# IlzeAmandaA/VAE-GP-ODE

Hardware: AMD Instinct MI355X
Metric: latent_trajectories_per_sec (higher is better)
Workload: dtype f32; 1 GPU; configs[1]: ode1 DF q=6 M=100 S=256 T=16 batch=256; step = full ELBO training step (encoder, GP draw, rk4 rollout, decoder, ELBO, backward, Adam), L=1; global_batch=256, mc_draws=1, solver=rk4 (3/8 rule), parallelism=dp1, hip_graph=True, graph_scope=whole, gp_side_stream=True, batchnorm=per-process statistics

## Files before the change

vae-gp-ode_amd/csrc/gp_cache.hip:

```cpp
#include <type_traits>
#include "gp_eval.hpp"
#include "gp_launch.hpp"
#include "wave_reduce.hpp"
#include "gp_ws.hpp"

namespace gp {

static constexpr float kJitter = 1e-5f;

__device__ __forceinline__ float softplus_lower(float x) {
  float sp = x > 20.f ? x : log1pf(expf(x));
  return sp + 1e-12f;
}

struct PrepArgs {
  int kernel, Di, Do, M, S;
  const float *raw_ell, *raw_var, *Z, *Um, *Us, *eps_u, *rff_w, *rff_eps, *rff_u;
  float *pack, *pack_ind, *uni;
  float *ell_ws, *var_ws, *u_ws;
  float *ell_out, *var_out, *omega_out, *phase_out, *u_out;
  int* info;
  int nb_rff, nb_u, nb_ind, nb_hyp, nb_om;
  size_t s_eps_u, s_rff_w, s_rff_eps, s_rff_u, s_pack;
};
// ... 228 lines not shown
  return bad;
}

__global__ __launch_bounds__(256) void k_chol_rl(float* __restrict__ Aall, float* __restrict__ Lall, int np,
                                                  size_t batch_stride, float* __restrict__ Dfac_all, size_t dfac_stride,
                                                  int k, int* __restrict__ info, int nblk, int jlim, int nreal) {
  __shared__ float sD[NB][NB + 1], sI[NB][NB + 1], sJ[NB][NB + 1];
  __shared__ float lD[NB][NB + 1], lI[NB][NB + 1], lJ[NB][NB + 1];
  float* A = Aall + (size_t)blockIdx.y * batch_stride;
  float* Lm = Lall + (size_t)blockIdx.y * batch_stride;
  float* Dfac = Dfac_all + (size_t)blockIdx.y * dfac_stride + (size_t)k * NB * NB;
  const int t = blockIdx.x;
  int i, j;
  if (jlim >= nblk) {
    int ii = (int)((sqrtf(8.f * (float)t + 1.f) - 1.f) * 0.5f);
    while ((ii + 1) * (ii + 2) / 2 <= t) ++ii;
    while (ii * (ii + 1) / 2 > t) --ii;
    i = k + ii; j = k + (t - ii * (ii + 1) / 2);
  } else {
    int rem = t;
    j = k;
    while (rem >= nblk - j) { rem -= nblk - j; ++j; }
    i = j + rem;
  }
  const bool hasI = i > k, hasJ = (j > k) && (j != i);
  const int tid = threadIdx.x, tx = tid & 31, ty = tid >> 5;
  const int c0 = k * NB;
#pragma unroll
  for (int q = 0; q < 4; ++q) {
    const int r = ty + 8 * q;
    sD[r][tx] = A[(size_t)(c0 + r) * np + c0 + tx];
    sI[r][tx] = hasI ? A[(size_t)(i * NB + r) * np + c0 + tx] : 0.f;
    sJ[r][tx] = hasJ ? A[(size_t)(j * NB + r) * np + c0 + tx] : 0.f;
  }
  __syncthreads();
  const int wv = tid >> 6, lane = tid & 63;
  if (wv == 0 || (wv == 1 && hasJ)) {
    const int r = lane & 31;
    const bool panel = lane >= 32;
    float row[NB];
#pragma unroll
    for (int c = 0; c < NB; ++c) row[c] = panel ? (wv == 0 ? sI[r][c] : sJ[r][c]) : sD[r][c];
    const bool bad = chol32_panel_wave(row);
    if (bad && wv == 0 && t == 0 && lane == 0) atomicOr(info, 1);
    float* dst = panel ? (wv == 0 ? &lI[r][0] : &lJ[r][0]) : &lD[r][0];
#pragma unroll
    for (int c = 0; c < NB; ++c) dst[c] = (panel || c <= r) ? row[c] : 0.f;
  }
  __syncthreads();
  if (j == k) {
#pragma unroll
    for (int q = 0; q < 4; ++q) {
      const int r = ty + 8 * q;
      if (i == k) {
        Dfac[r * NB + tx] = lD[r][tx];
        if (r == tx && c0 + r < nreal) {
          atomicMin(reinterpret_cast<unsigned*>(info) + 1, __float_as_uint(lD[r][tx]));
          atomicMax(reinterpret_cast<unsigned*>(info) + 2, __float_as_uint(lD[r][tx]));
        }
      } else Lm[(size_t)(i * NB + r) * np + c0 + tx] = lI[r][tx];
    }
  } else {
#pragma unroll
    for (int q = 0; q < 4; ++q) {
      const int r = ty + 8 * q;
      float acc = 0.f;
      if (hasJ) {
#pragma unroll 8
        for (int p = 0; p < NB; ++p) acc = fmaf(lI[r][p], lJ[tx][p], acc);
      } else {
#pragma unroll 8
        for (int p = 0; p < NB; ++p) acc = fmaf(lI[r][p], lI[tx][p], acc);
      }
      float* dst = A + (size_t)(i * NB + r) * np + j * NB + tx;
      *dst = *dst - acc;
    }
  }
}

__device__ __forceinline__ void tile_load(float (&dst)[NB][NB + 1], const float* __restrict__ A, int np, int r0, int c0, int tx, int ty) {
#pragma unroll
  for (int q = 0; q < 4; ++q) dst[ty + 8 * q][tx] = A[(size_t)(r0 + ty + 8 * q) * np + c0 + tx];
}
__device__ __forceinline__ void tile_sub_xyt(float (&dst)[NB][NB + 1], const float (&src)[NB][NB + 1], const float (&X)[NB][NB + 1],
                                             const float (&Y)[NB][NB + 1], int tx, int ty) {
#pragma unroll
  for (int q = 0; q < 4; ++q) {
    const int r = ty + 8 * q;
    float acc = 0.f;
#pragma unroll 8
    for (int p = 0; p < NB; ++p) acc = fmaf(X[r][p], Y[tx][p], acc);
    dst[r][tx] = src[r][tx] - acc;
  }
}
__device__ __forceinline__ bool tile_factor(const float (&Dt)[NB][NB + 1], const float (&Pt)[NB][NB + 1], float (&Lp)[NB][NB + 1],
                                            float (*Ld)[NB + 1], int lane) {
  const int r = lane & 31;
  const bool panel = lane >= 32;
  float row[NB];
#pragma unroll
  for (int c = 0; c < NB; ++c) row[c] = panel ? Pt[r][c] : Dt[r][c];
  const bool bad = chol32_panel_wave(row);
  if (panel) {
#pragma unroll
    for (int c = 0; c < NB; ++c) Lp[r][c] = row[c];
  } else if (Ld) {
#pragma unroll
    for (int c = 0; c < NB; ++c) Ld[r][c] = c <= r ? row[c] : 0.f;
  }
  return bad;
}

__global__ __launch_bounds__(256) void k_chol_rl2(float* __restrict__ Aall, float* __restrict__ Lall, int np, size_t batch_stride,
                                                   float* __restrict__ Dfac_all, size_t dfac_stride, int k, int* __restrict__ info,
                                                   int nblk, int nreal) {
  __shared__ float sD[NB][NB + 1], sPi[NB][NB + 1], sPj[NB][NB + 1], sP1[NB][NB + 1];
  __shared__ float sE[NB][NB + 1], sQi[NB][NB + 1], sQj[NB][NB + 1];
  __shared__ float lD[NB][NB + 1], lPi[NB][NB + 1], lPj[NB][NB + 1], lP1[NB][NB + 1];
  __shared__ float lE[NB][NB + 1], lQi[NB][NB + 1], lQj[NB][NB + 1];
  float* A = Aall + (size_t)blockIdx.y * batch_stride;
  float* Lm = Lall + (size_t)blockIdx.y * batch_stride;
  float* DfacB = Dfac_all + (size_t)blockIdx.y * dfac_stride;
  const int t = blockIdx.x;
  int ii = (int)((sqrtf(8.f * (float)t + 1.f) - 1.f) * 0.5f);
  while ((ii + 1) * (ii + 2) / 2 <= t) ++ii;
  while (ii * (ii + 1) / 2 > t) --ii;
  const int i = k + ii, j = k + (t - ii * (ii + 1) / 2);
  const int k1 = k + 1;
  const int tid = threadIdx.x, tx = tid & 31, ty = tid >> 5, wv = tid >> 6, lane = tid & 63;
  const int c0 = k * NB, c1 = k1 * NB;
  const bool colk = j == k;
  const bool colk1 = j == k1;
  const bool needI = i > k, needJ = j > k && j != i;
  const bool need1 = !colk && i != k1 && j != k1;
  tile_load(sD, A, np, c0, c0, tx, ty);
  if (needI) tile_load(sPi, A, np, i * NB, c0, tx, ty);
  if (needJ) tile_load(sPj, A, np, j * NB, c0, tx, ty);
  if (need1) tile_load(sP1, A, np, c1, c0, tx, ty);
  if (!colk) {
    tile_load(sE, A, np, c1, c1, tx, ty);
    if (i > k1) tile_load(sQi, A, np, i * NB, c1, tx, ty);
    if (j > k1 && j != i) tile_load(sQj, A, np, j * NB, c1, tx, ty);
  }
  __syncthreads();
  bool bad = false;
  if (wv == 0) bad = tile_factor(sD, needI ? sPi : sD, lPi, lD, lane);
  else if (wv == 1 && needJ) tile_factor(sD, sPj, lPj, nullptr, lane);
  else if (wv == 2 && need1) tile_factor(sD, sP1, lP1, nullptr, lane);
  if (bad && t == 0 && lane == 0 && wv == 0) atomicOr(info, 1);
  __syncthreads();
  if (colk) {
#pragma unroll
    for (int q = 0; q < 4; ++q) {
      const int r = ty + 8 * q;
      if (i == k) {
        DfacB[(size_t)k * NB * NB + r * NB + tx] = lD[r][tx];
        if (r == tx && c0 + r < nreal) {
          atomicMin(reinterpret_cast<unsigned*>(info) + 1, __float_as_uint(lD[r][tx]));
          atomicMax(reinterpret_cast<unsigned*>(info) + 2, __float_as_uint(lD[r][tx]));
        }
      } else Lm[(size_t)(i * NB + r) * np + c0 + tx] = lPi[r][tx];
    }
    return;
  }
  const float (&L1)[NB][NB + 1] = (i == k1) ? lPi : ((j == k1) ? lPj : lP1);
  tile_sub_xyt(sE, sE, L1, L1, tx, ty);
  if (i > k1) tile_sub_xyt(sQi, sQi, lPi, L1, tx, ty);
  if (j > k1 && j != i) tile_sub_xyt(sQj, sQj, lPj, L1, tx, ty);
  __syncthreads();
  bool bad1 = false;
  if (wv == 0) bad1 = tile_factor(sE, i > k1 ? sQi : sE, lQi, lE, lane);
  else if (wv == 1 && j > k1 && j != i) tile_factor(sE, sQj, lQj, nullptr, lane);
  if (bad1 && t == 2 && lane == 0 && wv == 0) atomicOr(info, 1);
  __syncthreads();
  if (colk1) {
#pragma unroll
    for (int q = 0; q < 4; ++q) {
      const int r = ty + 8 * q;
      if (i == k1) {
        DfacB[(size_t)k1 * NB * NB + r * NB + tx] = lE[r][tx];
        if (r == tx && c1 + r < nreal) {
          atomicMin(reinterpret_cast<unsigned*>(info) + 1, __float_as_uint(lE[r][tx]));
          atomicMax(reinterpret_cast<unsigned*>(info) + 2, __float_as_uint(lE[r][tx]));
        }
      } else Lm[(size_t)(i * NB + r) * np + c1 + tx] = lQi[r][tx];
    }
    return;
  }
  const float (&Lj0)[NB][NB + 1] = (j == i) ? lPi : lPj;
  const float (&Lj1)[NB][NB + 1] = (j == i) ? lQi : lQj;
#pragma unroll
  for (int q = 0; q < 4; ++q) {
    const int r = ty + 8 * q;
    float acc = 0.f;
#pragma unroll 8
    for (int p = 0; p < NB; ++p) acc = fmaf(lPi[r][p], Lj0[tx][p], acc);
#pragma unroll 8
    for (int p = 0; p < NB; ++p) acc = fmaf(lQi[r][p], Lj1[tx][p], acc);
    float* dst = A + (size_t)(i * NB + r) * np + j * NB + tx;
    *dst = *dst - acc;
  }
}

typedef float cf32x4 __attribute__((ext_vector_type(4)));
constexpr int ST = 128, SK = 16, SLD = ST + 16;

__global__ __launch_bounds__(256, 2) void k_syrk_mfma(float* __restrict__ Aall, const float* __restrict__ Lall, int np,
                                                       size_t batch_stride, int r0, int c0) {
  __shared__ __attribute__((aligned(16))) float sA[SK][SLD], sB[SK][SLD];
  float* A = Aall + (size_t)blockIdx.y * batch_stride;
  const float* Lm = Lall + (size_t)blockIdx.y * batch_stride;
  const int t = blockIdx.x;
  int tm = (int)((sqrtf(8.f * (float)t + 1.f) - 1.f) * 0.5f);
  while ((tm + 1) * (tm + 2) / 2 <= t) ++tm;
  while (tm * (tm + 1) / 2 > t) --tm;
  const int tn = t - tm * (tm + 1) / 2;
  const int tid = threadIdx.x, lane = tid & 63, wave = tid >> 6, lr = lane & 15, lk = lane >> 4;
  const int wm = (wave & 1) * 64, wn = (wave >> 1) * 64;
  cf32x4 acc[4][4];
#pragma unroll
  for (int i = 0; i < 4; ++i)
#pragma unroll
    for (int j = 0; j < 4; ++j) acc[i][j] = cf32x4{0.f, 0.f, 0.f, 0.f};
  const float* Pa = Lm + ((size_t)r0 + (size_t)tm * ST) * np + c0;
  const float* Pb = Lm + ((size_t)r0 + (size_t)tn * ST) * np + c0;
  float4 ra[2], rb[2];
  auto load = [&](int kt) {
#pragma unroll
    for (int q = 0; q < 2; ++q) {
      const int e = tid + 256 * q, m = e >> 2, k4 = (e & 3) * 4;
      ra[q] = *reinterpret_cast<const float4*>(&Pa[(size_t)m * np + kt * SK + k4]);
      rb[q] = *reinterpret_cast<const float4*>(&Pb[(size_t)m * np + kt * SK + k4]);
    }
  };
  load(0);
  for (int kt = 0; kt < ST / SK; ++kt) {
    __syncthreads();
#pragma unroll
    for (int q = 0; q < 2; ++q) {
      const int e = tid + 256 * q, m = e >> 2, k4 = (e & 3) * 4;
      sA[k4 + 0][m] = ra[q].x; sA[k4 + 1][m] = ra[q].y; sA[k4 + 2][m] = ra[q].z; sA[k4 + 3][m] = ra[q].w;
      sB[k4 + 0][m] = rb[q].x; sB[k4 + 1][m] = rb[q].y; sB[k4 + 2][m] = rb[q].z; sB[k4 + 3][m] = rb[q].w;
    }
    __syncthreads();
    if (kt + 1 < ST / SK) load(kt + 1);
#pragma unroll
    for (int ks = 0; ks < SK / 4; ++ks) {
      float af[4], bf[4];
#pragma unroll
      for (int i = 0; i < 4; ++i) { af[i] = sA[4 * ks + lk][wm + 16 * i + lr]; bf[i] = sB[4 * ks + lk][wn + 16 * i + lr]; }
#pragma unroll
      for (int i = 0; i < 4; ++i)
#pragma unroll
        for (int j = 0; j < 4; ++j) acc[i][j] = __builtin_amdgcn_mfma_f32_16x16x4f32(af[i], bf[j], acc[i][j], 0, 0, 0);
    }
  }
  float* C = A + ((size_t)r0 + (size_t)tm * ST) * np + r0 + (size_t)tn * ST;
#pragma unroll
  for (int i = 0; i < 4; ++i)
#pragma unroll
    for (int j = 0; j < 4; ++j)
#pragma unroll
      for (int r = 0; r < 4; ++r) {
        float* dst = C + (size_t)(wm + 16 * i + 4 * lk + r) * np + wn + 16 * j + lr;
        *dst = *dst - acc[i][j][r];
      }
}

template <int CP4>
__global__ __launch_bounds__(256) void k_solve_back(const float* __restrict__ Aall, int n, int np, size_t batch_stride,
                                                     const float* __restrict__ Dfac_all, size_t dfac_stride,
                                                     const float* __restrict__ u, int u_stride, int u_bstride,
                                                     float* __restrict__ nu, float* __restrict__ nu_out,
                                                     int kernel, int Di, int Do, int M, const float* __restrict__ var,
                                                     float* __restrict__ pack_ind, size_t u_dstride, size_t nu_dstride,
                                                     size_t pack_dstride) {
  extern __shared__ __attribute__((aligned(16))) float sv[];
  __shared__ float sx[NB];
  const int b = blockIdx.x, dr = blockIdx.y;
  const float* A = Aall + (size_t)b * batch_stride;
  const float* Dfac = Dfac_all + (size_t)b * dfac_stride;
  u += (size_t)dr * u_dstride;
  nu += (size_t)dr * nu_dstride;
// ... 487 lines not shown
  }
  if (c != P) {
    if (half == 0) y[col] = res;
    return;
  }
  float colv[PW];
  const int g0 = P * PW;
  if (half == 0) {
#pragma unroll
    for (int r = 0; r < PW; ++r) colv[r] = (r >= tid && g0 + r < n) ? factor_elem(Lm, Dfac, np, g0 + r, g0 + tid) : 0.f;
  }
  __syncthreads();
#pragma unroll
  for (int r = PW - 1; r >= 0; --r) {
    if (tid == r) {
      const float x = (g0 + r < n) ? res / colv[r] : 0.f;
      sx[r] = x;
      res = x;
    }
    __syncthreads();
    if (tid < r) res = fmaf(-colv[r], sx[r], res);
  }
  if (half == 0 && col < n) nub[col] = res;
}

__global__ void k_nu_publish(int n, const float* __restrict__ nu, float* __restrict__ nu_out, int kernel, int Di, int Do,
                             const float* __restrict__ var, float* __restrict__ pack_ind, size_t nu_dstride, size_t pack_dstride) {
  const int b = blockIdx.y, j = blockIdx.x * blockDim.x + threadIdx.x;
  if (j >= n) return;
  nu += (size_t)blockIdx.z * nu_dstride;
  if (nu_out) nu_out += (size_t)blockIdx.z * nu_dstride;
  pack_ind += (size_t)blockIdx.z * pack_dstride;
  const float v = nu[(size_t)b * n + j];
  if (nu_out) nu_out[(size_t)b * n + j] = v;
  if (!pack_ind) return;
  const int RQ2 = cdiv(Di + Do, 4);
  int m, d;
  float coef;
  if (kernel == 0) { m = j; d = b; coef = var[d] * v; } else { m = j / Do; d = j % Do; coef = v; }
  const int field = Di + d;
  pack_ind[(((size_t)(m >> 6) * RQ2 + (field >> 2)) * 64 + (m & 63)) * 4 + (field & 3)] = coef;
}

__global__ void k_fill_from_K(int kernel, int Do, int n, int np, const float* __restrict__ Ku, const float* __restrict__ u_prior,
                              float* __restrict__ A) {
  const int c = blockIdx.x * blockDim.x + threadIdx.x;
  const int r = blockIdx.y, b = blockIdx.z;
  if (c >= np) return;
  float v;
  if (r < n && c < n) v = Ku[((size_t)b * n + r) * n + c] + (r == c ? kJitter : 0.f);
  else if (r == n) v = c < n ? (kernel == 0 ? u_prior[(size_t)c * Do + b] : u_prior[c]) : (c == n ? 1e30f : 0.f);
  else v = (r == c) ? 1.f : 0.f;
  A[((size_t)b * np + r) * np + c] = v;
}

__global__ void k_copy_L(const float* __restrict__ Aall, const float* __restrict__ Dfac_all, size_t dinv_stride,
                         int n, int np, size_t batch_stride, float* __restrict__ Lu) {
  const int c = blockIdx.x * blockDim.x + threadIdx.x;
  const int r = blockIdx.y, b = blockIdx.z;
  if (c >= n) return;
  float v = 0.f;
  if (c <= r) {
    const int kb = r / NB;
    v = (c < kb * NB) ? Aall[(size_t)b * batch_stride + (size_t)r * np + c]
                      : Dfac_all[(size_t)b * dinv_stride + ((size_t)kb * NB + (r - kb * NB)) * NB + (c - kb * NB)];
  }
  Lu[((size_t)b * n + r) * n + c] = v;
}

static size_t pack_floats_for(int kernel, int Di, int Do, int M, int S) {
  const size_t SJ = cdiv(S, 64), MJ = cdiv(M, 64);
  if (kernel == 0) return 256 * (SJ * Do * cdiv(Di + 2, 4) + MJ * cdiv(Di + Do, 4)) + (size_t)cdiv(Do * Di, 4) * 4;
  return 256 * (SJ * Do * cdiv(2 * Do + 3, 4) + MJ * cdiv(2 * Do, 4)) + (size_t)cdiv(2 * Do * Do + Do, 4) * 4;
}

int cache_sizes(int kernel, int Di, int Do, int M, int S, size_t* pack_floats, size_t* ws_floats, int nd) {
  if (!dims_supported(kernel, Di, Do)) return set_error("gpode_cache_sizes: no specialisation for kernel=%d Di=%d Do=%d", kernel, Di, Do);
  if (M < 1 || S < 1 || nd < 1) return set_error("gpode_cache_sizes: M=%d S=%d draws=%d", M, S, nd);
  if (pack_floats) *pack_floats = pack_floats_for(kernel, Di, Do, M, S);
  if (ws_floats) *ws_floats = ws_layout(kernel, Di, Do, M, S, nd).total;
  return 0;
}

static void cholesky_blocked(float* A, float* Lmat, float* Dfac, int np, int nblk, int batch, int* info, hipStream_t st, int nreal) {
  struct { int np, nblk, batch; } w{np, nblk, batch};
  const size_t bstride = (size_t)np * np, dstride = (size_t)nblk * NB * NB;
  constexpr int PB = ST / NB;
  if (big_factor(w.np)) {
    for (int K = 0; K < w.nblk / PB; ++K) {
      const int jlim = (K + 1) * PB;
      for (int k = K * PB; k < jlim; ++k) {
        int tiles = 0;
        for (int j = k; j < jlim; ++j) tiles += w.nblk - j;
        hipLaunchKernelGGL(k_chol_rl, dim3(tiles, w.batch), 256, 0, st, A, Lmat, w.np, bstride, Dfac, dstride, k, info, w.nblk, jlim, nreal);
      }
      const int Tt = w.nblk / PB - (K + 1);
      if (Tt > 0)
        hipLaunchKernelGGL(k_syrk_mfma, dim3(Tt * (Tt + 1) / 2, w.batch), 256, 0, st, A, Lmat, w.np, bstride, jlim * NB, K * ST);
    }
  } else {
    int k = 0;
    for (; k + 1 < w.nblk; k += 2) {
      const int T = w.nblk - k;
      hipLaunchKernelGGL(k_chol_rl2, dim3(T * (T + 1) / 2, w.batch), 256, 0, st, A, Lmat, w.np, bstride, Dfac, dstride, k, info, w.nblk, nreal);
    }
    for (; k < w.nblk; ++k) {
      const int T = w.nblk - k;
      hipLaunchKernelGGL(k_chol_rl, dim3(T * (T + 1) / 2, w.batch), 256, 0, st, A, Lmat, w.np, bstride, Dfac, dstride, k, info, w.nblk, w.nblk, nreal);
    }
  }
}

int cache_build_fwd(int kernel, int Di, int Do, int M, int S, int nd,
                    const float* raw_ell, const float* raw_var, const float* Z, const float* Um, const float* Us_packed,
                    const float* eps_u, const float* rff_w, const float* rff_eps, const float* rff_u,
                    float* pack, float* ws, float* ell, float* var, float* omega, float* phase, float* u,
                    float* Lu, float* nu, float* u_prior, hipStream_t st) {
  if (!dims_supported(kernel, Di, Do)) return set_error("gpode_cache_build_fwd: no specialisation for kernel=%d Di=%d Do=%d", kernel, Di, Do);
  if (kernel == 1 && Di != Do) return set_error("gpode_cache_build_fwd: DF needs D_in == D_out (kernels.py:259-262)");
  if (nd < 1 || nd > 65535) return set_error("gpode_cache_build_fwd: %d draws", nd);
  const WsLayout w = ws_layout(kernel, Di, Do, M, S, nd);
  const size_t SJ = cdiv(S, 64), MJ = cdiv(M, 64);
  const size_t rff_f4 = (kernel == 0 ? SJ * Do * cdiv(Di + 2, 4) : SJ * Do * cdiv(2 * Do + 3, 4)) * 64;
  const size_t ind_f4 = (kernel == 0 ? MJ * cdiv(Di + Do, 4) : MJ * cdiv(2 * Do, 4)) * 64;
  const size_t pf = pack_floats_for(kernel, Di, Do, M, S);
  const size_t MD = (size_t)M * Do;
  float* pack_ind = pack + 4 * rff_f4;
  float* uni = pack + 4 * (rff_f4 + ind_f4);
  int* info = reinterpret_cast<int*>(ws + w.info);
  {
    PrepArgs a;
    a.kernel = kernel; a.Di = Di; a.Do = Do; a.M = M; a.S = S;
    a.raw_ell = raw_ell; a.raw_var = raw_var; a.Z = Z; a.Um = Um; a.Us = Us_packed;
    a.eps_u = eps_u; a.rff_w = rff_w; a.rff_eps = rff_eps; a.rff_u = rff_u;
    a.pack = pack; a.pack_ind = pack_ind; a.uni = uni;
    a.ell_ws = ws + w.ell; a.var_ws = ws + w.var; a.u_ws = ws + w.u;
    a.ell_out = ell; a.var_out = var; a.omega_out = omega; a.phase_out = phase; a.u_out = u;
    a.info = info;
    a.nb_rff = cdiv((int)(SJ * Do * 64), 256);
    a.nb_u = cdiv(M * Do, 4);
    a.nb_ind = cdiv((int)(MJ * 64), 256);
    a.nb_hyp = 1;
    a.nb_om = (omega || phase) ? cdiv(Di * S * Do, 256) : 0;
    a.s_eps_u = MD; a.s_rff_w = (size_t)(kernel == 0 ? S : 2 * S) * Do; a.s_rff_eps = (size_t)Di * S * Do; a.s_rff_u = (size_t)S * Do;
    a.s_pack = pf;
    hipLaunchKernelGGL(k_prep, dim3(a.nb_rff + a.nb_u + a.nb_ind + a.nb_hyp + a.nb_om, nd), 256, 0, st, a);
    if (check_launch("cache prep")) return 1;
  }

  float* up = u_prior ? u_prior : ws + w.u_prior;
  if (rhs_fwd(kernel, Di, Do, M, S, pack, Z, M, up, 1, st, Draws{nd, pf, 0, MD})) return 1;

  float* A = ws + w.A;
  float* Lmat = ws + w.Lmat;
  float* Dfac = ws + w.Dfac;
  const size_t bstride = (size_t)w.np * w.np, dstride = (size_t)w.nblk * NB * NB;
  if (draw_in_lds(w.np, M, Di, nd)) {
    const size_t lds = draw_lds_bytes(w.np, M, Di, nd);
    if (kernel == 0) {
      if (set_max_lds((const void*)k_draw_lds<0>, lds)) return 1;
      hipLaunchKernelGGL(k_draw_lds<0>, w.batch, 512, lds, st, Di, Do, M, w.n, w.np, w.nblk, Z, ws + w.ell, ws + w.var, up, ws + w.u, Lmat,
                         bstride, Dfac, dstride, ws + w.nu, nu, pack_ind, info, nd, MD, MD, pf);
    } else {
      if (set_max_lds((const void*)k_draw_lds<1>, lds)) return 1;
      hipLaunchKernelGGL(k_draw_lds<1>, w.batch, 512, lds, st, Di, Do, M, w.n, w.np, w.nblk, Z, ws + w.ell, ws + w.var, up, ws + w.u, Lmat,
                         bstride, Dfac, dstride, ws + w.nu, nu, pack_ind, info, nd, MD, MD, pf);
    }
    if (Lu) hipLaunchKernelGGL(k_copy_L, dim3(cdiv(w.n, 128), w.n, w.batch), 128, 0, st, Lmat, Dfac, dstride, w.n, w.np, bstride, Lu);
    return check_launch("cache build: lds");
  }
  if (kernel == 0)
    hipLaunchKernelGGL(k_Kzz_rbf, dim3(cdiv(w.np, 128), w.np, Do), 128, 0, st, Di, Do, M, w.np, Z, ws + w.ell, ws + w.var, up, A, nd);
  else
    hipLaunchKernelGGL(k_Kzz_df, dim3(cdiv(w.np, 128), w.np, 1), 128, 0, st, Do, M, w.np, Z, ws + w.ell, ws + w.var, up, A, nd);
  cholesky_blocked(A, Lmat, Dfac, w.np, w.nblk, w.batch, info, st, w.n);
  if (check_launch("cholesky")) return 1;

  const int u_stride = kernel == 0 ? Do : 1, u_bstride = kernel == 0 ? 1 : 0;
  const char* route = "cache build: panel";
  if (big_factor(w.np)) {
    const int npanel = cdiv(w.n, ST);
    for (int P = npanel - 1; P >= 0; --P)
      hipLaunchKernelGGL(k_solve_back_panel, dim3(P + 1, w.batch, nd), 256, 0, st, Lmat, w.n, w.np, bstride, Dfac, dstride, ws + w.u,
                         u_stride, u_bstride, A, ws + w.nu, P, P == npanel - 1 ? 1 : 0, MD, MD);
    hipLaunchKernelGGL(k_nu_publish, dim3(cdiv(w.n, 256), w.batch, nd), 256, 0, st, w.n, ws + w.nu, nu, kernel, Di, Do, ws + w.var, pack_ind,
                       MD, pf);
  } else {
    if (solve_back_deep_fits(w.np, w.nblk)) {
      const size_t ldsd = sizeof(float) * ((size_t)w.np + (size_t)w.nblk * NB * NB);
      if (set_max_lds((const void*)k_solve_back_deep, ldsd)) return 1;
      hipLaunchKernelGGL(k_solve_back_deep, dim3(w.batch, nd), SBD_THREADS, ldsd, st, Lmat, w.n, w.np, bstride, Dfac, dstride, ws + w.u,
                         u_stride, u_bstride, ws + w.nu, nu, kernel, Di, Do, M, ws + w.var, pack_ind, MD, MD, pf);
      if (Lu) hipLaunchKernelGGL(k_copy_L, dim3(cdiv(w.n, 128), w.n, w.batch), 128, 0, st, Lmat, Dfac, dstride, w.n, w.np, bstride, Lu);
      return check_launch("cache build: chain32+deep");
    }
    const size_t lds = sizeof(float) * w.np;
    const int cpt = cdiv(w.n, 1024);
#define GP_SOLVE(CPT)                                                                                              \
  do {                                                                                                             \
    if (set_max_lds((const void*)k_solve_back<CPT>, lds)) return 1;                                                \
    hipLaunchKernelGGL(k_solve_back<CPT>, dim3(w.batch, nd), 256, lds, st, Lmat, w.n, w.np, bstride, Dfac, dstride, ws + w.u,   \
                       u_stride, u_bstride, ws + w.nu, nu, kernel, Di, Do, M, ws + w.var, pack_ind, MD, MD, pf);   \
  } while (0)
    if (cpt == 1) GP_SOLVE(1);
    else if (cpt == 2) GP_SOLVE(2);
    else GP_SOLVE(0);
#undef GP_SOLVE
    route = cpt == 1 ? "cache build: chain32+back<1>" : cpt == 2 ? "cache build: chain32+back<2>" : "cache build: chain32+back<0>";
  }
  if (Lu) hipLaunchKernelGGL(k_copy_L, dim3(cdiv(w.n, 128), w.n, w.batch), 128, 0, st, Lmat, Dfac, dstride, w.n, w.np, bstride, Lu);
  return check_launch(route);
}

size_t kern_scratch_floats(int kernel, int Di, int Do, int M, int S) {
  return pack_floats_for(kernel, Di, Do, M, S) + (size_t)cdiv(Do * Di + Do, 4) * 4;
}

static void kern_prep(int kernel, int Di, int Do, int M, int S, const float* raw_ell, const float* raw_var, const float* Z,
                      const float* rff_w, const float* rff_eps, const float* rff_u, float* pack, float* omega, float* phase, hipStream_t st) {
  const size_t SJ = cdiv(S, 64), MJ = cdiv(M, 64);
  const size_t rff_f4 = (kernel == 0 ? SJ * Do * cdiv(Di + 2, 4) : SJ * Do * cdiv(2 * Do + 3, 4)) * 64;
  const size_t ind_f4 = (kernel == 0 ? MJ * cdiv(Di + Do, 4) : MJ * cdiv(2 * Do, 4)) * 64;
  float* hyp = pack + pack_floats_for(kernel, Di, Do, M, S);
  PrepArgs a;
  a.kernel = kernel; a.Di = Di; a.Do = Do; a.M = M; a.S = S;
  a.raw_ell = raw_ell; a.raw_var = raw_var; a.Z = Z; a.Um = nullptr; a.Us = nullptr;
  a.eps_u = nullptr; a.rff_w = rff_w; a.rff_eps = rff_eps; a.rff_u = rff_u;
  a.pack = pack; a.pack_ind = pack + 4 * rff_f4; a.uni = pack + 4 * (rff_f4 + ind_f4);
  a.ell_ws = hyp; a.var_ws = hyp + (size_t)Do * Di; a.u_ws = nullptr;
  a.ell_out = nullptr; a.var_out = nullptr; a.omega_out = omega; a.phase_out = phase; a.u_out = nullptr;
  a.info = nullptr;
  a.nb_rff = cdiv((int)(SJ * Do * 64), 256);
  a.nb_u = 0;
  a.nb_ind = cdiv((int)(MJ * 64), 256);
  a.nb_hyp = 1;
  a.nb_om = (omega || phase) ? cdiv(Di * S * Do, 256) : 0;
  a.s_eps_u = a.s_rff_w = a.s_rff_eps = a.s_rff_u = a.s_pack = 0;
  hipLaunchKernelGGL(k_prep, dim3(a.nb_rff + a.nb_u + a.nb_ind + a.nb_hyp + a.nb_om, 1), 256, 0, st, a);
}

int kern_cache(int kernel, int Di, int Do, int S, const float* raw_ell, const float* raw_var, const float* rff_w, const float* rff_eps,
               const float* rff_u, float* pack, float* omega, float* phase, hipStream_t st) {
  if (!dims_supported(kernel, Di, Do)) return set_error("gpode_kern_cache: no specialisation for kernel=%d Di=%d Do=%d", kernel, Di, Do);
  if (S < 1) return set_error("gpode_kern_cache: S=%d", S);
  kern_prep(kernel, Di, Do, 0, S, raw_ell, raw_var, nullptr, rff_w, rff_eps, rff_u, pack, omega, phase, st);
  return check_launch("kern.build_cache");
}

int compute_nu_ws(int kernel, int Di, int Do, int M, size_t* ws_floats) {
  if (!dims_supported(kernel, Di, Do) || M < 1) return set_error("gpode_compute_nu: kernel=%d Di=%d Do=%d M=%d", kernel, Di, Do, M);
  *ws_floats = ws_layout(kernel, Di, Do, M, 1, 1).total;
  return 0;
}

int compute_nu(int kernel, int Di, int Do, int M, const float* Ku, const float* u_prior, const float* u, float* nu, float* ws, hipStream_t st) {
  size_t need = 0;
  if (compute_nu_ws(kernel, Di, Do, M, &need)) return 1;
  const WsLayout w = ws_layout(kernel, Di, Do, M, 1, 1);
  float* A = ws + w.A;
  float* Lmat = ws + w.Lmat;
  float* Dfac = ws + w.Dfac;
  int* info = reinterpret_cast<int*>(ws + w.info);
  const size_t bstride = (size_t)w.np * w.np, dstride = (size_t)w.nblk * NB * NB, MD = (size_t)M * Do;
  if (hipMemsetAsync(info, 0, 4 * sizeof(int), st) != hipSuccess) return set_error("gpode_compute_nu: memset failed");
  hipLaunchKernelGGL(k_fill_from_K, dim3(cdiv(w.np, 128), w.np, w.batch), 128, 0, st, kernel, Do, w.n, w.np, Ku, u_prior, A);
  cholesky_blocked(A, Lmat, Dfac, w.np, w.nblk, w.batch, info, st, w.n);
  if (check_launch("compute_nu: cholesky")) return 1;
  const int u_stride = kernel == 0 ? Do : 1, u_bstride = kernel == 0 ? 1 : 0;
  if (big_factor(w.np)) {
    const int npanel = cdiv(w.n, ST);
    for (int P = npanel - 1; P >= 0; --P)
      hipLaunchKernelGGL(k_solve_back_panel, dim3(P + 1, w.batch, 1), 256, 0, st, Lmat, w.n, w.np, bstride, Dfac, dstride, u,
                         u_stride, u_bstride, A, ws + w.nu, P, P == npanel - 1 ? 1 : 0, MD, MD);
    hipLaunchKernelGGL(k_nu_publish, dim3(cdiv(w.n, 256), w.batch, 1), 256, 0, st, w.n, ws + w.nu, nu, kernel, Di, Do, (const float*)nullptr,
                       (float*)nullptr, MD, (size_t)0);
  } else {
    if (solve_back_deep_fits(w.np, w.nblk)) {
      const size_t ldsd = sizeof(float) * ((size_t)w.np + (size_t)w.nblk * NB * NB);
      if (set_max_lds((const void*)k_solve_back_deep, ldsd)) return 1;
      hipLaunchKernelGGL(k_solve_back_deep, dim3(w.batch, 1), SBD_THREADS, ldsd, st, Lmat, w.n, w.np, bstride, Dfac, dstride, u, u_stride,
                         u_bstride, ws + w.nu, nu, kernel, Di, Do, M, (const float*)nullptr, (float*)nullptr, MD, MD, (size_t)0);
      return check_launch("kern.compute_nu: chain32+deep");
    }
    const size_t lds = sizeof(float) * w.np;
    if (set_max_lds((const void*)k_solve_back<0>, lds)) return 1;
    hipLaunchKernelGGL(k_solve_back<0>, dim3(w.batch, 1), 256, lds, st, Lmat, w.n, w.np, bstride, Dfac, dstride, u, u_stride, u_bstride,
                       ws + w.nu, nu, kernel, Di, Do, M, (const float*)nullptr, (float*)nullptr, MD, MD, (size_t)0);
    return check_launch("kern.compute_nu: chain32+back<0>");
  }
  return check_launch("kern.compute_nu: panel");
}

int f_update(int kernel, int Di, int Do, int M, const float* raw_ell, const float* raw_var, const float* x2, const float* nu,
             const float* x, int N, float* out, float* pack, hipStream_t st) {
  if (!dims_supported(kernel, Di, Do) || M < 1) return set_error("gpode_f_update: kernel=%d Di=%d Do=%d M=%d", kernel, Di, Do, M);
  kern_prep(kernel, Di, Do, M, 0, raw_ell, raw_var, x2, nullptr, nullptr, nullptr, pack, nullptr, nullptr, st);
  const size_t MJ = cdiv(M, 64);
  (void)MJ;
  float* pack_ind = pack;
  const float* var = pack + pack_floats_for(kernel, Di, Do, M, 0) + (size_t)Do * Di;
  const int n = kernel == 0 ? M : M * Do, batch = kernel == 0 ? Do : 1;
  hipLaunchKernelGGL(k_nu_publish, dim3(cdiv(n, 256), batch, 1), 256, 0, st, n, nu, (float*)nullptr, kernel, Di, Do, var, pack_ind,
                     (size_t)0, (size_t)0);
  if (check_launch("kern.f_update: pack")) return 1;
  return rhs_fwd(kernel, Di, Do, M, 0, pack, x, N, out, 2, st);
}

struct CondLayout { size_t info, A, Lmat, Dfac, a, t, total; int np, nblk; };
static CondLayout cond_layout(int Do, int M, int N) {
  CondLayout c;
  c.nblk = cdiv(M + N, NB);
  if (c.nblk >= 32) c.nblk = (c.nblk + 3) / 4 * 4;
  c.np = c.nblk * NB;
  size_t o = 0;
  auto take = [&](size_t nfl) { size_t at = o; o += (nfl + 3) / 4 * 4; return at; };
  c.info = take(4);
  c.A = take((size_t)Do * c.np * c.np);
  c.Lmat = take((size_t)Do * c.np * c.np);
  c.Dfac = take((size_t)Do * c.nblk * NB * NB);
  c.a = take((size_t)Do * N * M);
  c.t = take((size_t)Do * N * M);
  c.total = o;
  return c;
}

__device__ __forceinline__ float rbf_k(int Di, const float* __restrict__ raw_ell_d, float var_d, const float* __restrict__ p,
                                       const float* __restrict__ q) {
  float s = 0.f;
  for (int i = 0; i < Di; ++i) {
    const float t = (p[i] - q[i]) / softplus_lower(raw_ell_d[i]);
    s = fmaf(t, t, s);
  }
  return var_d * expf(-0.5f * s);
}

__global__ void k_cond_fill(int Di, int Do, int M, int N, int np, const float* __restrict__ raw_ell, const float* __restrict__ raw_var,
                            const float* __restrict__ Z, const float* __restrict__ x, float* __restrict__ A, int* __restrict__ info) {
  const int c = blockIdx.x * blockDim.x + threadIdx.x;
  const int r = blockIdx.y, d = blockIdx.z;
  if (c == 0 && r == 0 && d == 0) info[0] = 0;
  if (c >= np) return;
  const float vd = softplus_lower(raw_var[d]);
  float v;
  if (r < M) v = c < M ? rbf_k(Di, raw_ell + d * Di, vd, Z + (size_t)r * Di, Z + (size_t)c * Di) + (r == c ? kJitter : 0.f) : 0.f;
  else if (r < M + N) v = c < M ? rbf_k(Di, raw_ell + d * Di, vd, x + (size_t)(r - M) * Di, Z + (size_t)c * Di) : (c == r ? 1e30f : 0.f);
  else v = (r == c) ? 1.f : 0.f;
  A[((size_t)d * np + r) * np + c] = v;
}

// ... 11 lines not shown
  float* trow = Tws + ((size_t)d * N + n) * M;
  for (int m = tid; m < M; m += 256) {
    const float v = factor_elem(Lm, Dfac, np, M + n, m);
    sa[m] = v;
    arow[m] = v;
  }
  __syncthreads();
  float acc[3] = {0.f, 0.f, 0.f};
  if (us_rank1) {
    const float* sd = Us + (size_t)d * M;
    float part[1] = {0.f}, tot[1];
    for (int j = tid; j < M; j += 256) {
      part[0] = fmaf(sd[j], sa[j], part[0]);
      acc[0] = fmaf(sa[j], Um[(size_t)j * Do + d], acc[0]);
      acc[2] = fmaf(sa[j], sa[j], acc[2]);
      trow[j] = 0.f;
    }
    wave_sum_multi<1>(part, tot);
    if ((tid & 63) == 0) red[tid >> 6][0] = tot[0];
    __syncthreads();
    const float t0 = (red[0][0] + red[1][0]) + (red[2][0] + red[3][0]);
    __syncthreads();
    if (tid == 0) { trow[0] = t0; acc[1] = t0 * t0; }
  } else {
    const float* Ud = Us + (size_t)d * ((size_t)M * (M + 1) / 2);
    for (int j = tid; j < M; j += 256) {
      float t = 0.f;
      for (int m = j; m < M; ++m) t = fmaf(Ud[(size_t)m * (m + 1) / 2 + j], sa[m], t);
      trow[j] = t;
      acc[0] = fmaf(sa[j], Um[(size_t)j * Do + d], acc[0]);
      acc[1] = fmaf(t, t, acc[1]);
      acc[2] = fmaf(sa[j], sa[j], acc[2]);
    }
  }
  float out[3];
  wave_sum_multi<3>(acc, out);
  if ((tid & 63) == 0) { red[tid >> 6][0] = out[0]; red[tid >> 6][1] = out[1]; red[tid >> 6][2] = out[2]; }
  __syncthreads();
  if (tid == 0) {
    const float m0 = (red[0][0] + red[1][0]) + (red[2][0] + red[3][0]);
    const float t2 = (red[0][1] + red[1][1]) + (red[2][1] + red[3][1]);
    const float a2 = (red[0][2] + red[1][2]) + (red[2][2] + red[3][2]);
    mean[(size_t)n * Do + d] = m0;
    if (var_diag) var_diag[(size_t)n * Do + d] = softplus_lower(raw_var[d]) + (t2 - a2);
  }
}

__global__ __launch_bounds__(256) void k_cond_cov(int Di, int Do, int M, int N, const float* __restrict__ raw_ell,
                                                   const float* __restrict__ raw_var, const float* __restrict__ x,
                                                   const float* __restrict__ Aws, const float* __restrict__ Tws, float* __restrict__ cov) {
  const int lane = threadIdx.x & 63;
  const size_t pair = (size_t)blockIdx.x * 4 + (threadIdx.x >> 6);
  if (pair >= (size_t)N * N) return;
  const int n1 = (int)(pair / N), n2 = (int)(pair % N);
  for (int d = 0; d < Do; ++d) {
    const float* a1 = Aws + ((size_t)d * N + n1) * M;
    const float* a2 = Aws + ((size_t)d * N + n2) * M;
    const float* t1 = Tws + ((size_t)d * N + n1) * M;
    const float* t2 = Tws + ((size_t)d * N + n2) * M;
    float acc = 0.f;
    for (int m = lane; m < M; m += 64) acc += t1[m] * t2[m] - a1[m] * a2[m];
    const float in1[1] = {acc};
    float out1[1];
    wave_sum_multi<1>(in1, out1);
    if (lane == 0)
      cov[((size_t)n2 * N + n1) * Do + d] = rbf_k(Di, raw_ell + d * Di, softplus_lower(raw_var[d]), x + (size_t)n1 * Di, x + (size_t)n2 * Di) + out1[0];
  }
}

int conditional_ws(int Di, int Do, int M, int N, size_t* ws_floats) {
  if (Di <= 0 || Do <= 0 || M <= 0 || N <= 0) return set_error("gpode_conditional: Di=%d Do=%d M=%d N=%d", Di, Do, M, N);
  *ws_floats = cond_layout(Do, M, N).total;
  return 0;
}

int conditional(int Di, int Do, int M, int N, const float* raw_ell, const float* raw_var, const float* Z, const float* Um,
                const float* Us_packed, int us_rank1, const float* x, int full_cov, float* mean, float* var, float* ws, hipStream_t st) {
  size_t need = 0;
  if (conditional_ws(Di, Do, M, N, &need)) return 1;
  const CondLayout c = cond_layout(Do, M, N);
  int* info = reinterpret_cast<int*>(ws + c.info);
  const size_t bstride = (size_t)c.np * c.np, dstride = (size_t)c.nblk * NB * NB;
  hipLaunchKernelGGL(k_cond_fill, dim3(cdiv(c.np, 128), c.np, Do), 128, 0, st, Di, Do, M, N, c.np, raw_ell, raw_var, Z, x, ws + c.A, info);
  cholesky_blocked(ws + c.A, ws + c.Lmat, ws + c.Dfac, c.np, c.nblk, Do, info, st, M);
  if (check_launch("conditional: cholesky")) return 1;
  const size_t lds = sizeof(float) * M;
  if (set_max_lds((const void*)k_cond_rows, lds)) return 1;
  hipLaunchKernelGGL(k_cond_rows, dim3(N, Do), 256, lds, st, Do, M, N, c.np, ws + c.Lmat, bstride, ws + c.Dfac, dstride, raw_var, Um,
                     Us_packed, us_rank1, ws + c.a, ws + c.t, mean, full_cov ? nullptr : var);
  if (full_cov)
    hipLaunchKernelGGL(k_cond_cov, (unsigned)(((size_t)N * N + 3) / 4), 256, 0, st, Di, Do, M, N, raw_ell, raw_var, x, ws + c.a, ws + c.t, var);
  return check_launch(big_factor(c.np) ? "conditional: panel" : "conditional: chain32");
}

}
```

Before: 106,600 trajectories/s.

## Add four-column fused right-looking Cholesky kernel to cut launches

Adds k_chol_rl4, which factors four 32-wide block columns per launch. It stages the needed tiles in shared memory and runs the panel factor, strip updates and trailing update inside one 512-thread block, where the old path used two-column launches. Tile update loops are also register-blocked so each lane accumulates a small output block from float4/float2 shared-memory reads. The goal is fewer sequential kernel launches and less global-memory round-tripping in the small-matrix DF Cholesky, at the cost of more LDS per block, redundant panel work in every block, and more complex code. An env var can restore the two-column path.

```diff
diff --git a/vae-gp-ode_amd/csrc/gp_cache.hip b/vae-gp-ode_amd/csrc/gp_cache.hip
--- a/vae-gp-ode_amd/csrc/gp_cache.hip
+++ b/vae-gp-ode_amd/csrc/gp_cache.hip
@@ -334,16 +334,24 @@
 #pragma unroll
   for (int q = 0; q < 4; ++q) dst[ty + 8 * q][tx] = A[(size_t)(r0 + ty + 8 * q) * np + c0 + tx];
 }
+template <int ROWS, int NTY>
+__device__ __forceinline__ void tile_acc(float (&acc)[ROWS], const float (&X)[NB][NB + 1], const float (&Y)[NB][NB + 1], int tx, int ty) {
+  float y[NB];
+#pragma unroll
+  for (int p = 0; p < NB; ++p) y[p] = Y[tx][p];
+#pragma unroll
+  for (int q = 0; q < ROWS; ++q) {
+    const int r = ty + NTY * q;
+#pragma unroll
+    for (int p = 0; p < NB; ++p) acc[q] = fmaf(X[r][p], y[p], acc[q]);
+  }
+}
 __device__ __forceinline__ void tile_sub_xyt(float (&dst)[NB][NB + 1], const float (&src)[NB][NB + 1], const float (&X)[NB][NB + 1],
                                              const float (&Y)[NB][NB + 1], int tx, int ty) {
-#pragma unroll
-  for (int q = 0; q < 4; ++q) {
-    const int r = ty + 8 * q;
-    float acc = 0.f;
-#pragma unroll 8
-    for (int p = 0; p < NB; ++p) acc = fmaf(X[r][p], Y[tx][p], acc);
-    dst[r][tx] = src[r][tx] - acc;
-  }
+  float acc[4] = {0.f, 0.f, 0.f, 0.f};
+  tile_acc<4, 8>(acc, X, Y, tx, ty);
+#pragma unroll
+  for (int q = 0; q < 4; ++q) dst[ty + 8 * q][tx] = src[ty + 8 * q][tx] - acc[q];
 }
 __device__ __forceinline__ bool tile_factor(const float (&Dt)[NB][NB + 1], const float (&Pt)[NB][NB + 1], float (&Lp)[NB][NB + 1],
                                             float (*Ld)[NB + 1], int lane) {
@@ -441,16 +449,198 @@
   }
   const float (&Lj0)[NB][NB + 1] = (j == i) ? lPi : lPj;
   const float (&Lj1)[NB][NB + 1] = (j == i) ? lQi : lQj;
+  float acc[4] = {0.f, 0.f, 0.f, 0.f};
+  tile_acc<4, 8>(acc, lPi, Lj0, tx, ty);
+  tile_acc<4, 8>(acc, lQi, Lj1, tx, ty);
 #pragma unroll
   for (int q = 0; q < 4; ++q) {
-    const int r = ty + 8 * q;
-    float acc = 0.f;
+    float* dst = A + (size_t)(i * NB + ty + 8 * q) * np + j * NB + tx;
+    *dst = *dst - acc[q];
+  }
+}
+
+constexpr int RL4_THREADS = 512, RL4_TILES = 19, RL4_TILE = NB * (NB + 1);
+constexpr size_t RL4_LDS = sizeof(float) * RL4_TILES * RL4_TILE;
+typedef float chol_tile[NB][NB + 1];
+__device__ __forceinline__ int rl4_tile(int s, int c) { return s < 4 ? s * (s + 1) / 2 + c : 10 + 4 * (s - 4) + c; }
+
+__device__ __forceinline__ bool tile_factor_t(const chol_tile& Dt, chol_tile& Pt, float (*Ld)[NB + 1], float (*Lrow)[NB + 1], int lane) {
+  const int r = lane & 31;
+  const bool panel = lane >= 32;
+  float row[NB];
+#pragma unroll
+  for (int c = 0; c < NB; ++c) row[c] = panel ? Pt[r][c] : Dt[r][c];
+  const bool bad = chol32_panel_wave(row);
+  if (panel) {
+    float* Pf = &Pt[0][0];
+#pragma unroll
+    for (int c = 0; c < NB; ++c) Pf[c * NB + r] = row[c];
+    if (Lrow) {
+#pragma unroll
+      for (int c = 0; c < NB; ++c) Lrow[r][c] = row[c];
+    }
+  } else if (Ld) {
+#pragma unroll
+    for (int c = 0; c < NB; ++c) Ld[r][c] = c <= r ? row[c] : 0.f;
+  }
+  return bad;
+}
+
+__device__ __forceinline__ void strip_acc(float (&acc)[2][4], const chol_tile& Xt, const chol_tile& Yt, int h, int lane) {
+  const float2* xp = reinterpret_cast<const float2*>(&Xt[0][0] + 16 * h + 2 * (lane >> 3));
+  const float4* yp = reinterpret_cast<const float4*>(&Yt[0][0] + 4 * (lane & 7));
+#pragma unroll
+  for (int p = 0; p < NB; ++p) {
+    const float2 x = xp[p * (NB / 2)];
+    const float4 y = yp[p * (NB / 4)];
+    acc[0][0] = fmaf(x.x, y.x, acc[0][0]); acc[0][1] = fmaf(x.x, y.y, acc[0][1]);
+    acc[0][2] = fmaf(x.x, y.z, acc[0][2]); acc[0][3] = fmaf(x.x, y.w, acc[0][3]);
+    acc[1][0] = fmaf(x.y, y.x, acc[1][0]); acc[1][1] = fmaf(x.y, y.y, acc[1][1]);
+    acc[1][2] = fmaf(x.y, y.z, acc[1][2]); acc[1][3] = fmaf(x.y, y.w, acc[1][3]);
+  }
+}
+__device__ __forceinline__ void strip_sub(chol_tile& T, const float (&acc)[2][4], int h, int lane) {
+  const int r0 = 16 * h + 2 * (lane >> 3), c0 = 4 * (lane & 7);
+#pragma unroll
+  for (int q = 0; q < 2; ++q)
+#pragma unroll
+    for (int e = 0; e < 4; ++e) T[r0 + q][c0 + e] = T[r0 + q][c0 + e] - acc[q][e];
+}
+
+__device__ __forceinline__ void block_acc(float (&acc)[4][4], const chol_tile& Xt, const chol_tile& Yt, int lane) {
+  const float4* xp = reinterpret_cast<const float4*>(&Xt[0][0] + 4 * (lane >> 3));
+  const float4* yp = reinterpret_cast<const float4*>(&Yt[0][0] + 4 * (lane & 7));
 #pragma unroll 8
-    for (int p = 0; p < NB; ++p) acc = fmaf(lPi[r][p], Lj0[tx][p], acc);
-#pragma unroll 8
-    for (int p = 0; p < NB; ++p) acc = fmaf(lQi[r][p], Lj1[tx][p], acc);
-    float* dst = A + (size_t)(i * NB + r) * np + j * NB + tx;
-    *dst = *dst - acc;
+  for (int p = 0; p < NB; ++p) {
+    const float4 x = xp[p * (NB / 4)];
+    const float4 y = yp[p * (NB / 4)];
+    const float xs[4] = {x.x, x.y, x.z, x.w}, ys[4] = {y.x, y.y, y.z, y.w};
+#pragma unroll
+    for (int q = 0; q < 4; ++q)
+#pragma unroll
+      for (int e = 0; e < 4; ++e) acc[q][e] = fmaf(xs[q], ys[e], acc[q][e]);
+  }
+}
+__device__ __forceinline__ void block_sub(chol_tile& T, const float (&acc)[4][4], int lane) {
+  const int r0 = 4 * (lane >> 3), c0 = 4 * (lane & 7);
+#pragma unroll
+  for (int q = 0; q < 4; ++q)
+#pragma unroll
+    for (int e = 0; e < 4; ++e) T[r0 + q][c0 + e] = T[r0 + q][c0 + e] - acc[q][e];
+}
+
+__global__ __launch_bounds__(RL4_THREADS) void k_chol_rl4(float* __restrict__ Aall, float* __restrict__ Lall, int np, size_t batch_stride,
+                                                           float* __restrict__ Dfac_all, size_t dfac_stride, int k, int* __restrict__ info,
+                                                           int nblk, int nreal) {
+  extern __shared__ __attribute__((aligned(16))) float rl4_lds[];
+  chol_tile* tiles = reinterpret_cast<chol_tile*>(rl4_lds);
+  chol_tile& extra = tiles[RL4_TILES - 1];
+  float* A = Aall + (size_t)blockIdx.y * batch_stride;
+  float* Lm = Lall + (size_t)blockIdx.y * batch_stride;
+  float* DfacB = Dfac_all + (size_t)blockIdx.y * dfac_stride;
+  const int t = blockIdx.x;
+  int ii = (int)((sqrtf(8.f * (float)t + 1.f) - 1.f) * 0.5f);
+  while ((ii + 1) * (ii + 2) / 2 <= t) ++ii;
+  while (ii * (ii + 1) / 2 > t) --ii;
+  const int i = k + ii, j = k + (t - ii * (ii + 1) / 2);
+  const int tid = threadIdx.x, tx = tid & 31, ty = tid >> 5, wv = tid >> 6, lane = tid & 63;
+  const int si = i < k + 4 ? i - k : 4;
+  const int sj = j < k + 4 ? j - k : (j == i ? 4 : 5);
+  const int jc = j - k < 3 ? j - k : 3;
+  const unsigned mask = ((2u << jc) - 1u) | (1u << si) | (1u << sj);
+  const bool trailing = j > k + 3;
+  {
+    float v[RL4_TILES][2];
+#pragma unroll
+    for (int tt = 0; tt < RL4_TILES; ++tt) {
+      const int s = tt >= 18 ? 6 : tt >= 14 ? 5 : tt >= 10 ? 4 : tt >= 6 ? 3 : tt >= 3 ? 2 : tt >= 1 ? 1 : 0;
+      const int c = s >= 4 ? (tt - 10) & 3 : tt - s * (s + 1) / 2;
+      const bool need = s == 6 ? trailing : ((mask >> s & 1) && c <= jc);
+      const int row = s == 6 ? i : (s < 4 ? k + s : (s == 4 ? i : j));
+      const int col = s == 6 ? j : k + c;
+#pragma unroll
+      for (int q = 0; q < 2; ++q) v[tt][q] = need ? A[(size_t)(row * NB + ty + 16 * q) * np + col * NB + tx] : 0.f;
+    }
+#pragma unroll
+    for (int tt = 0; tt < RL4_TILES; ++tt)
+#pragma unroll
+      for (int q = 0; q < 2; ++q) tiles[tt][ty + 16 * q][tx] = v[tt][q];
+  }
+  __syncthreads();
+#pragma unroll 1
+  for (int c = 0; c < 4; ++c) {
+    const bool publisher = si == c && sj == c;
+    const bool last = j == k + c;
+    {
+      int ps = -1, cnt = 0;
+      for (int s = c + 1; s < 6; ++s)
+        if (mask >> s & 1) { if (cnt == wv) ps = s; ++cnt; }
+      if (wv == 0 || ps >= 0) {
+        const bool bad = tile_factor_t(tiles[rl4_tile(c, c)], tiles[rl4_tile(ps >= 0 ? ps : c, c)], (wv == 0 && publisher) ? &extra[0] : nullptr,
+                                       (last && ps == si) ? &extra[0] : nullptr, lane);
+        if (bad && publisher && wv == 0 && lane == 0) atomicOr(info, 1);
+      }
+    }
+    __syncthreads();
+    if (last) {
+      const int cc = (k + c) * NB;
+#pragma unroll
+      for (int q = 0; q < 2; ++q) {
+        const int r = ty + 16 * q;
+        if (publisher) {
+          DfacB[(size_t)(k + c) * NB * NB + r * NB + tx] = extra[r][tx];
+          if (r == tx && cc + r < nreal) {
+            atomicMin(reinterpret_cast<unsigned*>(info) + 1, __float_as_uint(extra[r][tx]));
+            atomicMax(reinterpret_cast<unsigned*>(info) + 2, __float_as_uint(extra[r][tx]));
+          }
+        } else Lm[(size_t)(i * NB + r) * np + cc + tx] = extra[r][tx];
+      }
+      return;
+    }
+    int u = 0;
+    if (c == 0 || c == 2) {
+      for (int s = c + 1; s < 6; ++s) {
+        if (!(mask >> s & 1)) continue;
+        for (int h = 0; h < 2; ++h, ++u) {
+          if ((u & 7) != wv) continue;
+          float acc[2][4] = {};
+          strip_acc(acc, tiles[rl4_tile(s, c)], tiles[rl4_tile(c + 1, c)], h, lane);
+          strip_sub(tiles[rl4_tile(s, c + 1)], acc, h, lane);
+        }
+      }
+    } else if (c == 1) {
+      for (int d = 2; d <= jc; ++d)
+        for (int s = d; s < 6; ++s) {
+          if (!(mask >> s & 1)) continue;
+          if ((u++ & 7) != wv) continue;
+          float acc[4][4] = {};
+          block_acc(acc, tiles[rl4_tile(s, 0)], tiles[rl4_tile(d, 0)], lane);
+          block_acc(acc, tiles[rl4_tile(s, 1)], tiles[rl4_tile(d, 1)], lane);
+          block_sub(tiles[rl4_tile(s, d)], acc, lane);
+        }
+      if (trailing && (u & 7) == wv) {
+        float acc[4][4] = {};
+        block_acc(acc, tiles[rl4_tile(si, 0)], tiles[rl4_tile(sj, 0)], lane);
+        block_acc(acc, tiles[rl4_tile(si, 1)], tiles[rl4_tile(sj, 1)], lane);
+        block_sub(extra, acc, lane);
+      }
+    } else {
+      if (wv < 2) {
+        float acc[2][4] = {};
+        strip_acc(acc, tiles[rl4_tile(si, 2)], tiles[rl4_tile(sj, 2)], wv, lane);
+        strip_acc(acc, tiles[rl4_tile(si, 3)], tiles[rl4_tile(sj, 3)], wv, lane);
+        const int r0 = 16 * wv + 2 * (lane >> 3), c0 = 4 * (lane & 7);
+#pragma unroll
+        for (int q = 0; q < 2; ++q) {
+          float4 v;
+          v.x = extra[r0 + q][c0] - acc[q][0]; v.y = extra[r0 + q][c0 + 1] - acc[q][1];
+          v.z = extra[r0 + q][c0 + 2] - acc[q][2]; v.w = extra[r0 + q][c0 + 3] - acc[q][3];
+          *reinterpret_cast<float4*>(A + (size_t)(i * NB + r0 + q) * np + j * NB + c0) = v;
+        }
+      }
+      return;
+    }
+    __syncthreads();
   }
 }
 
@@ -1104,7 +1294,7 @@
   return 0;
 }
 
-static void cholesky_blocked(float* A, float* Lmat, float* Dfac, int np, int nblk, int batch, int* info, hipStream_t st, int nreal) {
+static int cholesky_blocked(float* A, float* Lmat, float* Dfac, int np, int nblk, int batch, int* info, hipStream_t st, int nreal) {
   struct { int np, nblk, batch; } w{np, nblk, batch};
   const size_t bstride = (size_t)np * np, dstride = (size_t)nblk * NB * NB;
   constexpr int PB = ST / NB;
@@ -1121,7 +1311,16 @@
         hipLaunchKernelGGL(k_syrk_mfma, dim3(Tt * (Tt + 1) / 2, w.batch), 256, 0, st, A, Lmat, w.np, bstride, jlim * NB, K * ST);
     }
   } else {
+    static const bool cols2 = [] { const char* e = getenv("GPODE_CHOL_COLS"); return e && e[0] == '2'; }();
     int k = 0;
+    if (!cols2 && w.nblk >= 4) {
+      if (set_max_lds((const void*)k_chol_rl4, RL4_LDS)) return 1;
+      for (; k + 3 < w.nblk; k += 4) {
+        const int T = w.nblk - k;
+        hipLaunchKernelGGL(k_chol_rl4, dim3(T * (T + 1) / 2, w.batch), RL4_THREADS, RL4_LDS, st, A, Lmat, w.np, bstride, Dfac, dstride, k, info, w.nblk,
+                           nreal);
+      }
+    }
     for (; k + 1 < w.nblk; k += 2) {
       const int T = w.nblk - k;
       hipLaunchKernelGGL(k_chol_rl2, dim3(T * (T + 1) / 2, w.batch), 256, 0, st, A, Lmat, w.np, bstride, Dfac, dstride, k, info, w.nblk, nreal);
@@ -1131,6 +1330,7 @@
       hipLaunchKernelGGL(k_chol_rl, dim3(T * (T + 1) / 2, w.batch), 256, 0, st, A, Lmat, w.np, bstride, Dfac, dstride, k, info, w.nblk, w.nblk, nreal);
     }
   }
+  return 0;
 }
 
 int cache_build_fwd(int kernel, int Di, int Do, int M, int S, int nd,
@@ -1195,7 +1395,7 @@
     hipLaunchKernelGGL(k_Kzz_rbf, dim3(cdiv(w.np, 128), w.np, Do), 128, 0, st, Di, Do, M, w.np, Z, ws + w.ell, ws + w.var, up, A, nd);
   else
     hipLaunchKernelGGL(k_Kzz_df, dim3(cdiv(w.np, 128), w.np, 1), 128, 0, st, Do, M, w.np, Z, ws + w.ell, ws + w.var, up, A, nd);
-  cholesky_blocked(A, Lmat, Dfac, w.np, w.nblk, w.batch, info, st, w.n);
+  if (cholesky_blocked(A, Lmat, Dfac, w.np, w.nblk, w.batch, info, st, w.n)) return 1;
   if (check_launch("cholesky")) return 1;
 
   const int u_stride = kernel == 0 ? Do : 1, u_bstride = kernel == 0 ? 1 : 0;
@@ -1286,7 +1486,7 @@
   const size_t bstride = (size_t)w.np * w.np, dstride = (size_t)w.nblk * NB * NB, MD = (size_t)M * Do;
   if (hipMemsetAsync(info, 0, 4 * sizeof(int), st) != hipSuccess) return set_error("gpode_compute_nu: memset failed");
   hipLaunchKernelGGL(k_fill_from_K, dim3(cdiv(w.np, 128), w.np, w.batch), 128, 0, st, kernel, Do, w.n, w.np, Ku, u_prior, A);
-  cholesky_blocked(A, Lmat, Dfac, w.np, w.nblk, w.batch, info, st, w.n);
+  if (cholesky_blocked(A, Lmat, Dfac, w.np, w.nblk, w.batch, info, st, w.n)) return 1;
   if (check_launch("compute_nu: cholesky")) return 1;
   const int u_stride = kernel == 0 ? Do : 1, u_bstride = kernel == 0 ? 1 : 0;
   if (big_factor(w.np)) {
@@ -1464,7 +1664,7 @@
   int* info = reinterpret_cast<int*>(ws + c.info);
   const size_t bstride = (size_t)c.np * c.np, dstride = (size_t)c.nblk * NB * NB;
   hipLaunchKernelGGL(k_cond_fill, dim3(cdiv(c.np, 128), c.np, Do), 128, 0, st, Di, Do, M, N, c.np, raw_ell, raw_var, Z, x, ws + c.A, info);
-  cholesky_blocked(ws + c.A, ws + c.Lmat, ws + c.Dfac, c.np, c.nblk, Do, info, st, M);
+  if (cholesky_blocked(ws + c.A, ws + c.Lmat, ws + c.Dfac, c.np, c.nblk, Do, info, st, M)) return 1;
   if (check_launch("conditional: cholesky")) return 1;
   const size_t lds = sizeof(float) * M;
   if (set_max_lds((const void*)k_cond_rows, lds)) return 1;
```

Result: faster. 108,700 trajectories/s, median of 6 (+2.0%).
